# XuyangBai/D3Feat

Hardware: NVIDIA H100
Metric: points/sec through KPFCNN encoder (higher is better)
Workload: dtype f32

## Files before the change

d3feat_b200/csrc/kpconv.cu:

```cuda
#include <stdlib.h>

#include "ops.cuh"

namespace d3f {


constexpr int kS1Warps = 4;
constexpr int kWStride = 20;
constexpr int kKMax = 16;

struct Stage1Params {
  const float* q;
  const float4* s4;
  const int* idx;
  const float* feat;
  int count_nn;
  const float* Kp;
  const float* offsets;
  const float* modulations;
  int Nq, Ns, H, Cin;
  int n0, n1;
  const int* order;
  float extent;
  float inv_scale;
  float gauss_inv;
  int influence, closest;
  float shadow;
  float* wf;
  float* inv_nn;
  const int* nq_dev;
  const int* ns_dev;
};

__global__ void __launch_bounds__(256) prep_supports_kernel(const float* __restrict__ s, const float* __restrict__ feat,
                                                            int Ns_cap, const int* __restrict__ ns_dev, int Cin,
                                                            int mode, float shadow, float4* __restrict__ s4) {
  const int Ns = dyn_rows(Ns_cap, ns_dev);
  int warp = (blockIdx.x * blockDim.x + threadIdx.x) >> 5, lane = threadIdx.x & 31;
  if (warp > Ns) return;
  if (warp == Ns) {
    if (lane == 0) s4[Ns] = make_float4(shadow, shadow, shadow, 0.f);
    return;
  }
  float w = 0.f;
  if (mode == 1) {
    float sum = 0.f;
    for (int c = lane; c < Cin; c += 32) sum += feat[(size_t)warp * Cin + c];
#pragma unroll
    for (int o = 16; o > 0; o >>= 1) sum += __shfl_xor_sync(0xffffffffu, sum, o);
    w = sum > 0.f ? 1.f : 0.f;
  } else if (mode == 2) {
    w = feat[warp];
  }
  if (lane == 0) s4[warp] = make_float4(s[3 * (size_t)warp], s[3 * (size_t)warp + 1], s[3 * (size_t)warp + 2], w);
}

template <int G>
__global__ void __launch_bounds__(256) prep_supports_vec_kernel(const float* __restrict__ s,
                                                                const float* __restrict__ feat, int Ns_cap,
                                                                const int* __restrict__ ns_dev, int Cin,
                                                                float shadow, float4* __restrict__ s4) {
  const int Ns = dyn_rows(Ns_cap, ns_dev);
  const int t = blockIdx.x * blockDim.x + threadIdx.x;
  const int row = t / G, gl = t % G;
  float sum = 0.f;
  if (row < Ns) {
    const float4* fr = reinterpret_cast<const float4*>(feat + (size_t)row * Cin);
    for (int c4 = gl; c4 < Cin / 4; c4 += G) {
      float4 v = fr[c4];
      sum += (v.x + v.y) + (v.z + v.w);
    }
  }
#pragma unroll
  for (int o = G / 2; o > 0; o >>= 1) sum += __shfl_xor_sync(0xffffffffu, sum, o);
  if (gl == 0) {
    if (row < Ns)
      s4[row] = make_float4(s[3 * (size_t)row], s[3 * (size_t)row + 1], s[3 * (size_t)row + 2], sum > 0.f ? 1.f : 0.f);
    else if (row == Ns)
      s4[Ns] = make_float4(shadow, shadow, shadow, 0.f);
  }
}

template <int K, int VEC, bool DEFORM>
__global__ void __launch_bounds__(kS1Warps * 32) kpconv_stage1_kernel(Stage1Params p) {
  const int Ns_ = dyn_rows(p.Ns, p.ns_dev), n1_ = min(p.n1, dyn_rows(p.Nq, p.nq_dev));
  static_assert(K <= kKMax, "K too large");
  __shared__ __align__(16) float wts[kS1Warps][32 * kWStride];
  __shared__ float kp_s[kS1Warps][kKMax * 3];
  const int lane = threadIdx.x & 31, warp = threadIdx.x >> 5;
  const int n = p.n0 + blockIdx.x * kS1Warps + warp;
  if (n >= n1_) return;
  const int qid = p.order ? p.order[n] : n;

  for (int t = lane; t < K * 3; t += 32) {
    float v = p.Kp[t];
    if (DEFORM) v += p.offsets[(size_t)qid * K * 3 + t];
    kp_s[warp][t] = v;
  }
  for (int t = K * 3 + lane; t < kKMax * 3; t += 32) kp_s[warp][t] = 0.f;
  const float qx = p.q[3 * (size_t)qid], qy = p.q[3 * (size_t)qid + 1], qz = p.q[3 * (size_t)qid + 2];
  const int* row = p.idx + (size_t)qid * p.H;
  const float ext2 = p.extent * p.extent;
  __syncwarp();

  int nn_count = 0;
  const int c_step = 32 * VEC;
  for (int c0 = 0; c0 < p.Cin; c0 += c_step) {
    float acc[K][VEC];
#pragma unroll
    for (int k = 0; k < K; ++k)
#pragma unroll
      for (int v = 0; v < VEC; ++v) acc[k][v] = 0.f;
    const int c = c0 + lane * VEC;
    const bool c_ok = c < p.Cin;

    for (int h0 = 0; h0 < p.H; h0 += 32) {
      const int h = h0 + lane;
      int id = (h < p.H) ? row[h] : Ns_;
      if (id < 0 || id > Ns_) id = Ns_;
      const bool real = id < Ns_;
      const float4 sp = __ldg(&p.s4[id]);
      const float rx = sp.x - qx, ry = sp.y - qy, rz = sp.z - qz;
      float w[kKMax];
      float dmin = 3.0e38f;
      int kmin = 0;
      bool in_range = false;
#pragma unroll
      for (int k = 0; k < K; ++k) {
        float dx = rx - kp_s[warp][3 * k], dy = ry - kp_s[warp][3 * k + 1], dz = rz - kp_s[warp][3 * k + 2];
        float d2 = dx * dx + dy * dy + dz * dz;
        if (d2 < dmin) { dmin = d2; kmin = k; }
        in_range = in_range || (d2 < ext2);
        float wk;
        if (p.influence == D3F_INFLUENCE_LINEAR) wk = fmaxf(1.f - sqrtf(d2 + 1e-10f) * p.inv_scale, 0.f);
        else if (p.influence == D3F_INFLUENCE_GAUSSIAN) wk = expf(-d2 * p.gauss_inv);
        else wk = DEFORM ? (d2 < ext2 ? 1.f : 0.f) : 1.f;
        w[k] = wk;
      }
      if (p.closest) {
#pragma unroll
        for (int k = 0; k < K; ++k) w[k] = (k == kmin) ? w[k] : 0.f;
      }
      const bool keep = real && (!DEFORM || in_range);
#pragma unroll
      for (int k = 0; k < kKMax; ++k) wts[warp][lane * kWStride + k] = (keep && k < K) ? w[k] : 0.f;
      if (c0 == 0 && p.count_nn) nn_count += __popc(__ballot_sync(0xffffffffu, sp.w > 0.f));
      const unsigned keep_mask = __ballot_sync(0xffffffffu, keep);
      __syncwarp();

      unsigned m = keep_mask;
      while (m) {
        int hh[4];
        float f[4][VEC];
        int cnt = 0;
#pragma unroll
        for (int u = 0; u < 4; ++u) {
          if (m) {
            hh[u] = __ffs(m) - 1;
            m &= m - 1;
            ++cnt;
          } else {
            hh[u] = -1;
          }
        }
#pragma unroll
        for (int u = 0; u < 4; ++u) {
          if (hh[u] >= 0) {
            int idh = __shfl_sync(0xffffffffu, id, hh[u]);
            const float* fp = p.feat + (size_t)idh * p.Cin + c;
            if (VEC == 4) {
              float4 t = c_ok ? *reinterpret_cast<const float4*>(fp) : make_float4(0.f, 0.f, 0.f, 0.f);
              f[u][0] = t.x; f[u][1 % VEC] = t.y; f[u][2 % VEC] = t.z; f[u][3 % VEC] = t.w;
            } else if (VEC == 2) {
              float2 t = c_ok ? *reinterpret_cast<const float2*>(fp) : make_float2(0.f, 0.f);
              f[u][0] = t.x; f[u][1 % VEC] = t.y;
            } else {
              f[u][0] = c_ok ? *fp : 0.f;
            }
          }
        }
#pragma unroll
        for (int u = 0; u < 4; ++u) {
          if (hh[u] >= 0) {
            const float4* wp = reinterpret_cast<const float4*>(&wts[warp][hh[u] * kWStride]);
            float wv[kKMax];
#pragma unroll
            for (int kq = 0; kq < (K + 3) / 4; ++kq) {
              float4 t = wp[kq];
              wv[4 * kq] = t.x; wv[4 * kq + 1] = t.y; wv[4 * kq + 2] = t.z; wv[4 * kq + 3] = t.w;
            }
#pragma unroll
            for (int k = 0; k < K; ++k)
#pragma unroll
              for (int v = 0; v < VEC; ++v) acc[k][v] = fmaf(wv[k], f[u][v], acc[k][v]);
          }
        }
        (void)cnt;
      }
      __syncwarp();
    }

    if (c_ok) {
      float* dst = p.wf + (size_t)(n - p.n0) * K * p.Cin + c;
#pragma unroll
      for (int k = 0; k < K; ++k) {
        float mod = (DEFORM && p.modulations) ? p.modulations[(size_t)qid * K + k] : 1.f;
        if (VEC == 4) {
// ... 508 lines not shown
        mma_tf32(acc[i], ah, bl0, bl1);
      }
    }

    float* dst = p.wf + (size_t)(n - p.n0) * K * p.Cin + c0 + 2 * NT * t;
    const float modA = (DEFORM && p.modulations) ? p.modulations[(size_t)qid * K + kA] : 1.f;
    const float modB = (DEFORM && p.modulations && validB) ? p.modulations[(size_t)qid * K + kB] : 1.f;
#pragma unroll
    for (int v = 0; v < NT; v += 4) {
      *reinterpret_cast<float4*>(dst + (size_t)kA * p.Cin + v) =
          make_float4(acc[v][0] * modA, acc[v + 1][0] * modA, acc[v + 2][0] * modA, acc[v + 3][0] * modA);
      *reinterpret_cast<float4*>(dst + (size_t)kA * p.Cin + NT + v) =
          make_float4(acc[v][1] * modA, acc[v + 1][1] * modA, acc[v + 2][1] * modA, acc[v + 3][1] * modA);
      if (validB) {
        *reinterpret_cast<float4*>(dst + (size_t)kB * p.Cin + v) =
            make_float4(acc[v][2] * modB, acc[v + 1][2] * modB, acc[v + 2][2] * modB, acc[v + 3][2] * modB);
        *reinterpret_cast<float4*>(dst + (size_t)kB * p.Cin + NT + v) =
            make_float4(acc[v][3] * modB, acc[v + 1][3] * modB, acc[v + 2][3] * modB, acc[v + 3][3] * modB);
      }
    }
  }
  if (p.inv_nn != nullptr && lane == 0) p.inv_nn[n - p.n0] = 1.f / (float)max(nn_count, 1);
}

constexpr int kAnyKMax = 64;

template <bool DEFORM>
__global__ void __launch_bounds__(kS1Warps * 32) kpconv_stage1_anyk_kernel(Stage1Params p, int K) {
  const int Ns_ = dyn_rows(p.Ns, p.ns_dev), n1_ = min(p.n1, dyn_rows(p.Nq, p.nq_dev));
  extern __shared__ float anyk_smem[];
  const int lane = threadIdx.x & 31, warp = threadIdx.x >> 5;
  float* wts = anyk_smem + (size_t)warp * (K * 32 + K * 3);
  float* kp_s = wts + K * 32;
  const int n = p.n0 + blockIdx.x * kS1Warps + warp;
  if (n >= n1_) return;
  const int qid = p.order ? p.order[n] : n;
  for (int t = lane; t < K * 3; t += 32) {
    float v = p.Kp[t];
    if (DEFORM) v += p.offsets[(size_t)qid * K * 3 + t];
    kp_s[t] = v;
  }
  const float qx = p.q[3 * (size_t)qid], qy = p.q[3 * (size_t)qid + 1], qz = p.q[3 * (size_t)qid + 2];
  const int* row = p.idx + (size_t)qid * p.H;
  const float ext2 = p.extent * p.extent;
  float* dst = p.wf + (size_t)(n - p.n0) * K * p.Cin;
  __syncwarp();
  int nn_count = 0;
  for (int h0 = 0; h0 < p.H || h0 == 0; h0 += 32) {
    const int h = h0 + lane;
    int id = (h < p.H) ? row[h] : Ns_;
    if (id < 0 || id > Ns_) id = Ns_;
    const bool real = id < Ns_;
    const float4 sp = __ldg(&p.s4[id]);
    const float rx = sp.x - qx, ry = sp.y - qy, rz = sp.z - qz;
    float dmin = 3.0e38f;
    int kmin = 0;
    bool in_range = false;
    for (int k = 0; k < K; ++k) {
      float dx = rx - kp_s[3 * k], dy = ry - kp_s[3 * k + 1], dz = rz - kp_s[3 * k + 2];
      float d2 = dx * dx + dy * dy + dz * dz;
      if (d2 < dmin) { dmin = d2; kmin = k; }
      in_range = in_range || (d2 < ext2);
      float wk;
      if (p.influence == D3F_INFLUENCE_LINEAR) wk = fmaxf(1.f - sqrtf(d2 + 1e-10f) * p.inv_scale, 0.f);
      else if (p.influence == D3F_INFLUENCE_GAUSSIAN) wk = expf(-d2 * p.gauss_inv);
      else wk = DEFORM ? (d2 < ext2 ? 1.f : 0.f) : 1.f;
      wts[k * 32 + lane] = wk;
    }
    const bool keep = real && (!DEFORM || in_range);
    for (int k = 0; k < K; ++k) {
      float wk = wts[k * 32 + lane];
      if (p.closest && k != kmin) wk = 0.f;
      if (!keep) wk = 0.f;
      if (DEFORM && p.modulations) wk *= p.modulations[(size_t)qid * K + k];
      wts[k * 32 + lane] = wk;
    }
    if (p.count_nn) nn_count += __popc(__ballot_sync(0xffffffffu, sp.w > 0.f));
    const unsigned keep_mask = __ballot_sync(0xffffffffu, keep);
    __syncwarp();
    for (int c0 = 0; c0 < p.Cin; c0 += 32) {
      const int c = c0 + lane;
      const bool c_ok = c < p.Cin;
      for (int k = 0; k < K; ++k) {
        float acc = (h0 == 0 || !c_ok) ? 0.f : dst[(size_t)k * p.Cin + c];
        unsigned m = keep_mask;
        while (m) {
          const int j = __ffs(m) - 1;
          m &= m - 1;
          const int idj = __shfl_sync(0xffffffffu, id, j);
          if (c_ok) acc = fmaf(wts[k * 32 + j], p.feat[(size_t)idj * p.Cin + c], acc);
        }
        if (c_ok) dst[(size_t)k * p.Cin + c] = acc;
      }
    }
    __syncwarp();
  }
  if (p.inv_nn != nullptr && lane == 0) p.inv_nn[n - p.n0] = 1.f / (float)max(nn_count, 1);
}

template <bool DEFORM>
static int launch_stage1(int K, const Stage1Params& p, cudaStream_t stream) {
  int nq = p.n1 - p.n0;
  bool al16 = (reinterpret_cast<uintptr_t>(p.feat) & 15) == 0 && (reinterpret_cast<uintptr_t>(p.wf) & 15) == 0;
  if (K == 15 && al16 && (p.Cin == 32 || p.Cin == 64 || p.Cin % 128 == 0)) {
    const int blocks = ceil_div(nq, kS1Warps);
    const bool fast = p.influence == D3F_INFLUENCE_LINEAR && !p.closest;
    static const bool no_pared = [] { const char* v = getenv("D3F_S1_PARED"); return v != nullptr && v[0] == '0'; }();
    if (fast && !DEFORM && !no_pared && (long long)(p.Ns + 1) * p.Cin < (1ll << 31)) {
      const char* sv = getenv("D3F_S1_STAGED");
      const int staged = sv ? atoi(sv) : 0;
      const dim3 grid_wide(blocks, p.Cin >= 128 ? p.Cin / 64 : 1);
      if (staged) {
        if (p.Cin == 32) kpconv_stage1_staged_kernel<4><<<blocks, kS1Warps * 32, 0, stream>>>(p);
        else kpconv_stage1_staged_kernel<8><<<grid_wide, kS1Warps * 32, 0, stream>>>(p);
        D3F_LAUNCH_CHECK("kpconv_stage1_staged_kernel");
        return D3F_OK;
      }
      if (p.Cin == 32) kpconv_stage1_fast_kernel<4><<<blocks, kS1Warps * 32, 0, stream>>>(p);
      else kpconv_stage1_fast_kernel<8><<<grid_wide, kS1Warps * 32, 0, stream>>>(p);
      D3F_LAUNCH_CHECK("kpconv_stage1_fast_kernel");
      return D3F_OK;
    }
    if (fast) {
      if (p.Cin == 32) kpconv_stage1_mma_kernel<4, DEFORM, true><<<blocks, kS1Warps * 32, 0, stream>>>(p);
      else if (p.Cin == 64) kpconv_stage1_mma_kernel<8, DEFORM, true><<<blocks, kS1Warps * 32, 0, stream>>>(p);
      else kpconv_stage1_mma_kernel<16, DEFORM, true><<<blocks, kS1Warps * 32, 0, stream>>>(p);
    } else {
      if (p.Cin == 32) kpconv_stage1_mma_kernel<4, DEFORM, false><<<blocks, kS1Warps * 32, 0, stream>>>(p);
      else if (p.Cin == 64) kpconv_stage1_mma_kernel<8, DEFORM, false><<<blocks, kS1Warps * 32, 0, stream>>>(p);
      else kpconv_stage1_mma_kernel<16, DEFORM, false><<<blocks, kS1Warps * 32, 0, stream>>>(p);
    }
    D3F_LAUNCH_CHECK("kpconv_stage1_mma_kernel");
    return D3F_OK;
  }
  if (K == 15 && al16 && p.Cin % 64 == 0) {
    kpconv_stage1_v2_kernel<2, 1, DEFORM><<<ceil_div(nq, kS1Warps), kS1Warps * 32, 0, stream>>>(p);
  } else if (K == 15 && al16 && p.Cin % 32 == 0) {
    kpconv_stage1_v2_kernel<2, 2, DEFORM><<<ceil_div(nq, kS1Warps * 2), kS1Warps * 32, 0, stream>>>(p);
  } else if (K == 15) {
    kpconv_stage1_kernel<15, 1, DEFORM><<<ceil_div(nq, kS1Warps), kS1Warps * 32, 0, stream>>>(p);
  } else {
    const size_t smem = (size_t)kS1Warps * (K * 32 + K * 3) * sizeof(float);
    kpconv_stage1_anyk_kernel<DEFORM><<<ceil_div(nq, kS1Warps), kS1Warps * 32, smem, stream>>>(p, K);
  }
  D3F_LAUNCH_CHECK("kpconv_stage1_kernel");
  return D3F_OK;
}

struct Cin1Params {
  const float* q; const float4* s4; const int* idx; const float* Kp; const float* W;
  int Nq, Ns, H, Cout;
  float inv_scale, gauss_inv;
  int influence, closest, normalize;
  float shadow;
  const float* bn_scale; const float* bn_shift; const float* bias;
  float leaky_alpha;
  const int* order;
  float* out;
  const int* nq_dev; const int* ns_dev;
};

template <bool FAST>
__global__ void __launch_bounds__(256, 3) kpconv_cin1_kernel(Cin1Params p) {
  const int Ns_ = dyn_rows(p.Ns, p.ns_dev), Nq_ = dyn_rows(p.Nq, p.nq_dev);
  constexpr int K = 15;
  extern __shared__ float c1_smem[];
  float* Ws = c1_smem;
  float* kp_s = c1_smem + K * p.Cout;
  for (int t = threadIdx.x; t < K * p.Cout; t += blockDim.x) Ws[t] = p.W[t];
  for (int t = threadIdx.x; t < K * 3; t += blockDim.x) kp_s[t] = p.Kp[t];
  __syncthreads();
  const int lane = threadIdx.x & 31;
  const int sub = lane >> 3, sl = lane & 7;
  const int slot0 = ((blockIdx.x * blockDim.x + threadIdx.x) >> 5) * 4;
  if (slot0 >= Nq_) return;
  const int slot = slot0 + sub;
  const bool qvalid = slot < Nq_;
  const int n = p.order ? p.order[qvalid ? slot : slot0] : (qvalid ? slot : slot0);
  const float qx = p.q[3 * (size_t)n], qy = p.q[3 * (size_t)n + 1], qz = p.q[3 * (size_t)n + 2];
  const int* row = p.idx + (size_t)n * p.H;
  float wf[K];
#pragma unroll
  for (int k = 0; k < K; ++k) wf[k] = 0.f;
  int nn = 0;
  if (FAST) {
    float kp[K * 3];
#pragma unroll
    for (int i = 0; i < K * 3; ++i) kp[i] = kp_s[i];
    const float inv_scale = p.inv_scale;
    const unsigned Nsu = (unsigned)Ns_;
    unsigned id1 = Nsu, id2 = Nsu;
    if (sl < p.H) id1 = min((unsigned)__ldg(row + sl), Nsu);
    if (sl + 8 < p.H) id2 = min((unsigned)__ldg(row + sl + 8), Nsu);
    float4 sp_n = __ldg(&p.s4[id1]);
    for (int h = sl; h < p.H; h += 8) {
      const float4 sp = sp_n;
      sp_n = __ldg(&p.s4[id2]);
      id2 = Nsu;
      if (h + 16 < p.H) id2 = min((unsigned)__ldg(row + h + 16), Nsu);
      const float f = sp.w, rx = sp.x - qx, ry = sp.y - qy, rz = sp.z - qz;
      nn += f > 0.f ? 1 : 0;
#pragma unroll
      for (int k = 0; k < K; ++k) {
        const float dx = rx - kp[3 * k], dy = ry - kp[3 * k + 1], dz = rz - kp[3 * k + 2];
        const float d2 = fmaf(dz, dz, fmaf(dy, dy, fmaf(dx, dx, 1e-10f)));
        const float wk = fmaxf(fmaf(-sqrt_approx(d2), inv_scale, 1.f), 0.f);
        wf[k] = fmaf(wk, f, wf[k]);
      }
    }
  } else
  for (int h = sl; h < p.H; h += 8) {
    int id = row[h];
    if (id < 0 || id > Ns_) id = Ns_;
    const float4 sp = __ldg(&p.s4[id]);
    const float f = sp.w, rx = sp.x - qx, ry = sp.y - qy, rz = sp.z - qz;
    nn += f > 0.f ? 1 : 0;
    float w[K];
    float dmin = 3.0e38f;
    int kmin = 0;
#pragma unroll
    for (int k = 0; k < K; ++k) {
      float dx = rx - kp_s[3 * k], dy = ry - kp_s[3 * k + 1], dz = rz - kp_s[3 * k + 2];
      float d2 = dx * dx + dy * dy + dz * dz;
      if (d2 < dmin) { dmin = d2; kmin = k; }
      float wk;
      if (p.influence == D3F_INFLUENCE_LINEAR) wk = fmaxf(1.f - sqrt_approx(d2 + 1e-10f) * p.inv_scale, 0.f);
      else if (p.influence == D3F_INFLUENCE_GAUSSIAN) wk = __expf(-d2 * p.gauss_inv);
      else wk = 1.f;
      w[k] = wk;
    }
#pragma unroll
    for (int k = 0; k < K; ++k) wf[k] += (p.closest && k != kmin) ? 0.f : w[k] * f;
  }
#pragma unroll
  for (int o = 1; o < 8; o <<= 1) {
#pragma unroll
    for (int k = 0; k < K; ++k) wf[k] += __shfl_xor_sync(0xffffffffu, wf[k], o);
    nn += __shfl_xor_sync(0xffffffffu, nn, o);
  }
  if (!qvalid) return;
  const float inv_nn = p.normalize ? 1.f / (float)max(nn, 1) : 1.f;
  for (int c = sl; c < p.Cout; c += 8) {
    float y = 0.f;
#pragma unroll
    for (int k = 0; k < K; ++k) y = fmaf(wf[k], Ws[k * p.Cout + c], y);
    y *= inv_nn;
    if (p.bn_scale) y = fmaf(y, p.bn_scale[c], p.bn_shift[c]);
    if (p.bias) y += p.bias[c];
    if (p.leaky_alpha >= 0.f) y = y > 0.f ? y : y * p.leaky_alpha;
    p.out[(size_t)n * p.Cout + c] = y;
  }
}

struct AuxStream {
  cudaStream_t stream = nullptr;
  cudaEvent_t s1_done[2] = {nullptr, nullptr};
  cudaEvent_t gemm_done[2] = {nullptr, nullptr};
};
constexpr int kMaxDevices = 32;
struct AuxStreams {
  AuxStream dev[kMaxDevices];
  ~AuxStreams() {
    for (int d = 0; d < kMaxDevices; ++d) {
      if (dev[d].stream == nullptr) continue;
      int cur = 0;
      if (cudaGetDevice(&cur) != cudaSuccess || cudaSetDevice(d) != cudaSuccess) continue;
      for (int i = 0; i < 2; ++i) {
        cudaEventDestroy(dev[d].s1_done[i]);
        cudaEventDestroy(dev[d].gemm_done[i]);
      }
      cudaStreamDestroy(dev[d].stream);
      cudaSetDevice(cur);
    }
  }
};
static AuxStream* aux_stream() {
  static thread_local AuxStreams all;
  int dev = 0;
  if (cudaGetDevice(&dev) != cudaSuccess || dev < 0 || dev >= kMaxDevices) return nullptr;
  AuxStream& a = all.dev[dev];
  if (a.stream != nullptr) return &a;
  cudaStreamCaptureMode mode = cudaStreamCaptureModeRelaxed;
  cudaThreadExchangeStreamCaptureMode(&mode);
  AuxStream n;
  bool ok = cudaStreamCreateWithFlags(&n.stream, cudaStreamNonBlocking) == cudaSuccess;
  for (int i = 0; ok && i < 2; ++i)
    ok = cudaEventCreateWithFlags(&n.s1_done[i], cudaEventDisableTiming) == cudaSuccess &&
         cudaEventCreateWithFlags(&n.gemm_done[i], cudaEventDisableTiming) == cudaSuccess;
  cudaThreadExchangeStreamCaptureMode(&mode);
  if (!ok) return nullptr;
  a = n;
  return &a;
}

static int chunk_queries(int K, int Cin) {
  static const int forced = [] { const char* v = getenv("D3F_KPCONV_CHUNK"); return v ? atoi(v) : 0; }();
  if (forced >= 128) return forced / 128 * 128;
  const long long per = (long long)K * Cin * 4;
  long long n = (512ll << 20) / per;
  if (n < 1024) n = 1024;
  return (int)(n / 128 * 128);
}

int kpconv_chunk_queries(int K, int Cin) { return chunk_queries(K, Cin); }

int kpconv_prep_supports(bool deform, const float* s, const float* feat, int Ns, const int* ns_dev, int K, int Cin,
                         int normalize, float4* s4, cudaStream_t stream) {
  const bool norm = normalize != 0 && !deform;
  const bool first_layer = Cin == 1 && !deform && K == 15;
  int pmode = first_layer ? 2 : (norm ? 1 : 0);
  const float shadow = deform ? 1000.f : 1e6f;
  const bool vec = pmode == 1 && Cin % 4 == 0 && Cin >= 32 && (reinterpret_cast<uintptr_t>(feat) & 15) == 0;
  if (vec && Cin < 64)
    prep_supports_vec_kernel<8><<<ceil_div((Ns + 1) * 8, 256), 256, 0, stream>>>(s, feat, Ns, ns_dev, Cin, shadow, s4);
  else if (vec && Cin < 128)
    prep_supports_vec_kernel<16><<<ceil_div((Ns + 1) * 16, 256), 256, 0, stream>>>(s, feat, Ns, ns_dev, Cin, shadow, s4);
  else if (vec)
    prep_supports_vec_kernel<32><<<ceil_div((Ns + 1) * 32, 256), 256, 0, stream>>>(s, feat, Ns, ns_dev, Cin, shadow, s4);
  else
    prep_supports_kernel<<<ceil_div((Ns + 1) * 32, 256), 256, 0, stream>>>(s, feat, Ns, ns_dev, Cin, pmode, shadow, s4);
  D3F_LAUNCH_CHECK("prep_supports_kernel");
  return D3F_OK;
}

int kpconv_stage1_wf(const float* q, const float4* s4, const int* idx, const float* feat, const float* Kp, int Nq, int Ns,
                     int H, int K, int Cin, float extent, int influence, int mode, int n0, int n1, float* wf,
                     cudaStream_t stream, const int* nq_dev, const int* ns_dev) {
  Stage1Params p;
  p.q = q; p.s4 = s4; p.idx = idx; p.feat = feat; p.count_nn = 0;
  p.Kp = Kp; p.offsets = nullptr; p.modulations = nullptr;
  p.Nq = Nq; p.Ns = Ns; p.H = H; p.Cin = Cin;
  p.n0 = n0; p.n1 = n1;
  p.order = nullptr;
  p.extent = extent;
  p.inv_scale = 1.f / (2.f * extent);
  float sigma = extent * 0.3f;
  p.gauss_inv = 1.f / (2.f * sigma * sigma + 1e-9f);
  p.influence = influence;
  p.closest = mode == D3F_MODE_CLOSEST;
  p.shadow = 1e6f;
  p.wf = wf;
  p.inv_nn = nullptr;
  p.nq_dev = nq_dev; p.ns_dev = ns_dev;
  return launch_stage1<false>(K, p, stream);
}

struct KpconvWs {
  float* wf[2];
  float* nn[2];
  float4* s4;
  float* split;
  float* w_img;
};

static size_t kpconv_layout(int Nq, int Ns, int K, int Cin, int Cout, void* base, KpconvWs* w_out) {
  int chunk = chunk_queries(K, Cin);
  if (chunk > Nq) chunk = Nq > 0 ? Nq : 1;
  Carver cv(base);
  KpconvWs w;
  for (int b = 0; b < 2; ++b) w.wf[b] = cv.take<float>((size_t)chunk * K * Cin);
  for (int b = 0; b < 2; ++b) w.nn[b] = cv.take<float>(chunk);
  w.s4 = cv.take<float4>((size_t)Ns + 1);
  const size_t split_floats = tc_gemm_split_ws_floats(chunk, Cout, K * Cin);
  w.split = split_floats ? cv.take<float>(split_floats) : nullptr;
  w.w_img = cv.take<float>(kpconv_fused_image_floats());
  if (w_out != nullptr) *w_out = w;
  return cv.off;
}

int kpconv_forward_impl(bool deform, const float* q, const float* s, const int* idx, const float* feat,
                        const float* Kp, const float* offsets, const float* modulations, const float* W,
                        const float* W_packed, const int* query_order, int Nq, int Ns, int H, int K, int Cin, int Cout,
                        float extent,
                        int influence, int mode, int normalize,
                        const float* bn_scale, const float* bn_shift, const float* bias, float leaky_alpha,
                        float* out, void* workspace, size_t workspace_bytes, cudaStream_t stream,
                        const int* nq_dev, const int* ns_dev) {
  D3F_REQUIRE(Nq >= 0 && Ns >= 0 && H >= 0 && Cin >= 1 && Cout >= 1, D3F_ERR_INVALID,
              "kpconv: bad shape Nq=%d Ns=%d H=%d Cin=%d Cout=%d", Nq, Ns, H, Cin, Cout);
  D3F_REQUIRE(K >= 1 && K <= kAnyKMax, D3F_ERR_INVALID, "kpconv: num_kernel_points=%d outside [1, %d]", K, kAnyKMax);
  D3F_REQUIRE(influence >= 0 && influence <= 2, D3F_ERR_INVALID,
              "Unknown influence function type (config.KP_influence)");
  D3F_REQUIRE(mode == D3F_MODE_SUM || mode == D3F_MODE_CLOSEST, D3F_ERR_INVALID,
              "Unknown convolution mode. Should be 'closest' or 'sum'");
  D3F_REQUIRE(extent > 0.f, D3F_ERR_INVALID, "kpconv: KP_extent=%g", (double)extent);
  D3F_REQUIRE((bn_scale == nullptr) == (bn_shift == nullptr), D3F_ERR_INVALID, "kpconv: bn_scale/bn_shift mismatch");
  D3F_REQUIRE(!deform || offsets != nullptr || Nq == 0, D3F_ERR_INVALID, "kpconv_deform: offsets missing");
  KpconvWs w;
  const size_t need = kpconv_layout(Nq, Ns, K, Cin, Cout, workspace, &w);
  D3F_REQUIRE(need > 0 && workspace_bytes >= need, D3F_ERR_WORKSPACE, "kpconv: workspace too small");
  if (Nq == 0) return D3F_OK;
  int chunk = chunk_queries(K, Cin);
  if (chunk > Nq) chunk = Nq;
  float4* s4 = w.s4;
  const bool norm = normalize != 0 && !deform;
  {
    const int rc = kpconv_prep_supports(deform, s, feat, Ns, ns_dev, K, Cin, normalize, s4, stream);
    if (rc) return rc;
  }
  const size_t c1_smem = (size_t)(K * Cout + K * 3) * sizeof(float);
  if (Cin == 1 && !deform && K == 15 && c1_smem <= 48 * 1024) {
    Cin1Params c1;
    c1.q = q; c1.s4 = s4; c1.idx = idx; c1.Kp = Kp; c1.W = W;
    c1.Nq = Nq; c1.Ns = Ns; c1.H = H; c1.Cout = Cout;
    c1.inv_scale = 1.f / (2.f * extent);
    float sg = extent * 0.3f;
    c1.gauss_inv = 1.f / (2.f * sg * sg + 1e-9f);
    c1.influence = influence; c1.closest = mode == D3F_MODE_CLOSEST; c1.normalize = normalize != 0;
    c1.shadow = 1e6f;
    c1.bn_scale = bn_scale; c1.bn_shift = bn_shift; c1.bias = bias; c1.leaky_alpha = leaky_alpha;
    c1.order = query_order;
    c1.out = out;
    c1.nq_dev = nq_dev; c1.ns_dev = ns_dev;
    if (influence == D3F_INFLUENCE_LINEAR && mode == D3F_MODE_SUM)
      kpconv_cin1_kernel<true><<<ceil_div(ceil_div(Nq, 4) * 32, 256), 256, c1_smem, stream>>>(c1);
    else
      kpconv_cin1_kernel<false><<<ceil_div(ceil_div(Nq, 4) * 32, 256), 256, c1_smem, stream>>>(c1);
    D3F_LAUNCH_CHECK("kpconv_cin1_kernel");
    return D3F_OK;
  }
  if (!deform && W_packed != nullptr &&
      kpconv_fused_supported(Nq, H, K, Cin, Cout, influence, mode, feat, W, out, query_order)) {
    return kpconv_fused_forward(q, s4, idx, feat, Kp, W, w.w_img, Nq, Ns, H, Cout, extent, norm ? 1 : 0, bn_scale, bn_shift,
                                bias, leaky_alpha, out, stream, nq_dev, ns_dev);
  }
  Stage1Params p;
  p.q = q; p.s4 = s4; p.idx = idx; p.feat = feat; p.count_nn = norm ? 1 : 0;
  p.Kp = Kp; p.offsets = offsets; p.modulations = modulations;
  p.Nq = Nq; p.Ns = Ns; p.H = H; p.Cin = Cin;
  p.extent = extent;
  p.inv_scale = deform ? 1.f / extent : 1.f / (2.f * extent);
  float sigma = extent * 0.3f;
  p.gauss_inv = 1.f / (2.f * sigma * sigma + 1e-9f);
  p.influence = influence;
  p.closest = mode == D3F_MODE_CLOSEST;
  p.shadow = deform ? 1000.f : 1e6f;
  p.order = query_order;
  p.nq_dev = nq_dev; p.ns_dev = ns_dev;
  const int n_chunks = ceil_div(Nq, chunk);
  AuxStream* aux = n_chunks > 1 ? aux_stream() : nullptr;
  for (int ci = 0, n0 = 0; n0 < Nq; n0 += chunk, ++ci) {
    const int b = ci & 1;
    float* wf = w.wf[b];
    float* inv_nn = w.nn[b];
    p.wf = wf;
    p.inv_nn = norm ? inv_nn : nullptr;
    p.n0 = n0;
    p.n1 = min(Nq, n0 + chunk);
    if (aux && ci >= 2) D3F_CUDA(cudaStreamWaitEvent(stream, aux->gemm_done[b], 0));
    int rc = deform ? launch_stage1<true>(K, p, stream) : launch_stage1<false>(K, p, stream);
    if (rc) return rc;
    cudaStream_t gs = stream;
    if (aux) {
      D3F_CUDA(cudaEventRecord(aux->s1_done[b], stream));
      D3F_CUDA(cudaStreamWaitEvent(aux->stream, aux->s1_done[b], 0));
      gs = aux->stream;
    }
    Epilogue ep;
    ep.rowscale = norm ? inv_nn : nullptr;
    ep.bn_scale = bn_scale; ep.bn_shift = bn_shift; ep.bias = bias; ep.residual = nullptr;
    ep.leaky_alpha = leaky_alpha;
    ep.row_map = query_order ? query_order + n0 : nullptr;
    ep.m_dev = nq_dev; ep.m_off = n0;
    float* cbase = query_order ? out : out + (size_t)n0 * Cout;
    if (W_packed != nullptr && tc_gemm_supported(wf, K * Cin))
      rc = tc_gemm(wf, W_packed, cbase, p.n1 - n0, Cout, K * Cin, ep, gs, w.split);
    else
      rc = gemm_f32(wf, W, cbase, p.n1 - n0, Cout, K * Cin, ep, gs);
    if (rc) return rc;
    if (aux) D3F_CUDA(cudaEventRecord(aux->gemm_done[b], aux->stream));
  }
  if (aux) {
    D3F_CUDA(cudaStreamWaitEvent(stream, aux->gemm_done[0], 0));
    if (n_chunks > 1) D3F_CUDA(cudaStreamWaitEvent(stream, aux->gemm_done[1], 0));
  }
  return D3F_OK;
}

}

using namespace d3f;

extern "C" size_t d3f_kpconv_workspace_bytes(int Nq, int Ns, int H, int K, int Cin, int Cout) {
  (void)H;
  return kpconv_layout(Nq, Ns, K, Cin, Cout, nullptr, nullptr);
}

extern "C" int d3f_kpconv_forward(const float* q, const float* s, const int* idx, const float* feat, const float* Kp,
                                  const float* W, const float* W_packed, const int* query_order, int Nq, int Ns, int H,
                                  int K, int Cin, int Cout, float extent, int influence, int mode, int normalize,
                                  const float* bn_scale, const float* bn_shift, const float* bias, float leaky_alpha,
                                  float* out, void* workspace, size_t workspace_bytes, d3f_stream_t stream,
                                  const int* nq_dev, const int* ns_dev) {
  D3F_REQUIRE(Nq == 0 || (q && idx && Kp && W && out && workspace && (Ns == 0 || (s && feat))), D3F_ERR_INVALID,
              "d3f_kpconv_forward: null pointer");
  return kpconv_forward_impl(false, q, s, idx, feat, Kp, nullptr, nullptr, W, W_packed, query_order, Nq, Ns, H, K, Cin,
                             Cout, extent, influence, mode, normalize, bn_scale, bn_shift, bias, leaky_alpha, out,
                             workspace, workspace_bytes, (cudaStream_t)stream, nq_dev, ns_dev);
}

extern "C" int d3f_kpconv_deform_forward(const float* q, const float* s, const int* idx, const float* feat,
                                         const float* Kp, const float* offsets, const float* modulations,
                                         const float* W, const float* W_packed, const int* query_order, int Nq, int Ns,
                                         int H, int K, int Cin, int Cout, float extent, int influence, int mode,
                                         const float* bn_scale, const float* bn_shift, const float* bias,
                                         float leaky_alpha, float* out, void* workspace, size_t workspace_bytes,
                                         d3f_stream_t stream, const int* nq_dev, const int* ns_dev) {
  D3F_REQUIRE(Nq == 0 || (q && idx && Kp && W && out && workspace && offsets && (Ns == 0 || (s && feat))),
              D3F_ERR_INVALID, "d3f_kpconv_deform_forward: null pointer");
  return kpconv_forward_impl(true, q, s, idx, feat, Kp, offsets, modulations, W, W_packed, query_order, Nq, Ns, H, K,
                             Cin, Cout, extent, influence, mode, 0, bn_scale, bn_shift, bias, leaky_alpha, out,
                             workspace, workspace_bytes, (cudaStream_t)stream, nq_dev, ns_dev);
}
```

Before: 64.83 million.

## Restructure Cin=1 KPConv kernel as persistent grid with pipelined neighbor loads

The single-input-channel KPConv kernel becomes a persistent, grid-strided kernel sized to SM count. It prefetches the next query's neighbor indices and support points while the current query computes, and handles two neighbors per iteration. The warp reduction is replaced by a transpose-style shuffle reduce, followed by a shared-memory exchange. Weights are re-laid out in shared memory for float4 output computation and vectorized stores, larger Cout is allowed through opt-in shared memory, and a lightweight per-row prep kernel is added for the non-summing modes. The change adds register pressure and code complexity, and cudaGetDevice and cudaDeviceGetAttribute are now called on every launch.

```diff
diff --git a/d3feat_b200/csrc/kpconv.cu b/d3feat_b200/csrc/kpconv.cu
--- a/d3feat_b200/csrc/kpconv.cu
+++ b/d3feat_b200/csrc/kpconv.cu
@@ -32,9 +32,21 @@
   const int* ns_dev;
 };
 
+__global__ void __launch_bounds__(256) prep_supports_rows_kernel(const float* __restrict__ s,
+                                                                 const float* __restrict__ feat, int Ns_cap,
+                                                                 const int* __restrict__ ns_dev, int with_feat,
+                                                                 float shadow, float4* __restrict__ s4) {
+  const int Ns = dyn_rows(Ns_cap, ns_dev);
+  const int i = blockIdx.x * blockDim.x + threadIdx.x;
+  if (i < Ns)
+    s4[i] = make_float4(s[3 * (size_t)i], s[3 * (size_t)i + 1], s[3 * (size_t)i + 2], with_feat ? feat[i] : 0.f);
+  else if (i == Ns)
+    s4[Ns] = make_float4(shadow, shadow, shadow, 0.f);
+}
+
 __global__ void __launch_bounds__(256) prep_supports_kernel(const float* __restrict__ s, const float* __restrict__ feat,
                                                             int Ns_cap, const int* __restrict__ ns_dev, int Cin,
-                                                            int mode, float shadow, float4* __restrict__ s4) {
+                                                            float shadow, float4* __restrict__ s4) {
   const int Ns = dyn_rows(Ns_cap, ns_dev);
   int warp = (blockIdx.x * blockDim.x + threadIdx.x) >> 5, lane = threadIdx.x & 31;
   if (warp > Ns) return;
@@ -42,17 +54,13 @@
     if (lane == 0) s4[Ns] = make_float4(shadow, shadow, shadow, 0.f);
     return;
   }
-  float w = 0.f;
-  if (mode == 1) {
-    float sum = 0.f;
-    for (int c = lane; c < Cin; c += 32) sum += feat[(size_t)warp * Cin + c];
-#pragma unroll
-    for (int o = 16; o > 0; o >>= 1) sum += __shfl_xor_sync(0xffffffffu, sum, o);
-    w = sum > 0.f ? 1.f : 0.f;
-  } else if (mode == 2) {
-    w = feat[warp];
-  }
-  if (lane == 0) s4[warp] = make_float4(s[3 * (size_t)warp], s[3 * (size_t)warp + 1], s[3 * (size_t)warp + 2], w);
+  float sum = 0.f;
+  for (int c = lane; c < Cin; c += 32) sum += feat[(size_t)warp * Cin + c];
+#pragma unroll
+  for (int o = 16; o > 0; o >>= 1) sum += __shfl_xor_sync(0xffffffffu, sum, o);
+  if (lane == 0)
+    s4[warp] = make_float4(s[3 * (size_t)warp], s[3 * (size_t)warp + 1], s[3 * (size_t)warp + 2],
+                           sum > 0.f ? 1.f : 0.f);
 }
 
 template <int G>
@@ -867,7 +875,7 @@
   int Nq, Ns, H, Cout;
   float inv_scale, gauss_inv;
   int influence, closest, normalize;
-  float shadow;
+  int vec;
   const float* bn_scale; const float* bn_shift; const float* bias;
   float leaky_alpha;
   const int* order;
@@ -875,95 +883,212 @@
   const int* nq_dev; const int* ns_dev;
 };
 
+constexpr int kC1Warps = 8;
+constexpr int kC1Blocks = 4;
+constexpr int kC1MaxCout = 816;
+
+static inline size_t cin1_smem_floats(int K, int Cout) {
+  return (size_t)(Cout + 3) / 4 * 4 * K + 4 * K + kC1Warps * 64;
+}
+
+__device__ __forceinline__ float cin1_linear(float rx, float ry, float rz, const float4& kp, float inv_scale) {
+  const float dx = rx - kp.x, dy = ry - kp.y, dz = rz - kp.z;
+  const float d2 = fmaf(dz, dz, fmaf(dy, dy, fmaf(dx, dx, 1e-10f)));
+  return fmaxf(fmaf(-sqrt_approx(d2), inv_scale, 1.f), 0.f);
+}
+
 template <bool FAST>
-__global__ void __launch_bounds__(256, 3) kpconv_cin1_kernel(Cin1Params p) {
+__global__ void __launch_bounds__(kC1Warps * 32, kC1Blocks) kpconv_cin1_kernel(Cin1Params p) {
+  constexpr int K = 15;
   const int Ns_ = dyn_rows(p.Ns, p.ns_dev), Nq_ = dyn_rows(p.Nq, p.nq_dev);
-  constexpr int K = 15;
-  extern __shared__ float c1_smem[];
+  extern __shared__ __align__(16) float c1_smem[];
+  const int Cout = p.Cout, H = p.H;
   float* Ws = c1_smem;
-  float* kp_s = c1_smem + K * p.Cout;
-  for (int t = threadIdx.x; t < K * p.Cout; t += blockDim.x) Ws[t] = p.W[t];
-  for (int t = threadIdx.x; t < K * 3; t += blockDim.x) kp_s[t] = p.Kp[t];
+  float4* kp_s = reinterpret_cast<float4*>(c1_smem + (Cout + 3) / 4 * 4 * K);
+  for (int t = threadIdx.x; t < K * Cout; t += blockDim.x) {
+    const int k = t / Cout, c = t - k * Cout;
+    Ws[((c >> 2) * K + k) * 4 + (c & 3)] = p.W[t];
+  }
+  if (threadIdx.x < K)
+    kp_s[threadIdx.x] = make_float4(p.Kp[3 * threadIdx.x], p.Kp[3 * threadIdx.x + 1], p.Kp[3 * threadIdx.x + 2], 0.f);
   __syncthreads();
-  const int lane = threadIdx.x & 31;
+  const int lane = threadIdx.x & 31, warp = threadIdx.x >> 5;
   const int sub = lane >> 3, sl = lane & 7;
-  const int slot0 = ((blockIdx.x * blockDim.x + threadIdx.x) >> 5) * 4;
-  if (slot0 >= Nq_) return;
-  const int slot = slot0 + sub;
-  const bool qvalid = slot < Nq_;
-  const int n = p.order ? p.order[qvalid ? slot : slot0] : (qvalid ? slot : slot0);
-  const float qx = p.q[3 * (size_t)n], qy = p.q[3 * (size_t)n + 1], qz = p.q[3 * (size_t)n + 2];
-  const int* row = p.idx + (size_t)n * p.H;
-  float wf[K];
-#pragma unroll
-  for (int k = 0; k < K; ++k) wf[k] = 0.f;
-  int nn = 0;
-  if (FAST) {
-    float kp[K * 3];
-#pragma unroll
-    for (int i = 0; i < K * 3; ++i) kp[i] = kp_s[i];
-    const float inv_scale = p.inv_scale;
-    const unsigned Nsu = (unsigned)Ns_;
-    unsigned id1 = Nsu, id2 = Nsu;
-    if (sl < p.H) id1 = min((unsigned)__ldg(row + sl), Nsu);
-    if (sl + 8 < p.H) id2 = min((unsigned)__ldg(row + sl + 8), Nsu);
-    float4 sp_n = __ldg(&p.s4[id1]);
-    for (int h = sl; h < p.H; h += 8) {
-      const float4 sp = sp_n;
-      sp_n = __ldg(&p.s4[id2]);
-      id2 = Nsu;
-      if (h + 16 < p.H) id2 = min((unsigned)__ldg(row + h + 16), Nsu);
-      const float f = sp.w, rx = sp.x - qx, ry = sp.y - qy, rz = sp.z - qz;
-      nn += f > 0.f ? 1 : 0;
-#pragma unroll
-      for (int k = 0; k < K; ++k) {
-        const float dx = rx - kp[3 * k], dy = ry - kp[3 * k + 1], dz = rz - kp[3 * k + 2];
-        const float d2 = fmaf(dz, dz, fmaf(dy, dy, fmaf(dx, dx, 1e-10f)));
-        const float wk = fmaxf(fmaf(-sqrt_approx(d2), inv_scale, 1.f), 0.f);
-        wf[k] = fmaf(wk, f, wf[k]);
-      }
-    }
-  } else
-  for (int h = sl; h < p.H; h += 8) {
-    int id = row[h];
-    if (id < 0 || id > Ns_) id = Ns_;
-    const float4 sp = __ldg(&p.s4[id]);
-    const float f = sp.w, rx = sp.x - qx, ry = sp.y - qy, rz = sp.z - qz;
-    nn += f > 0.f ? 1 : 0;
-    float w[K];
-    float dmin = 3.0e38f;
-    int kmin = 0;
-#pragma unroll
-    for (int k = 0; k < K; ++k) {
-      float dx = rx - kp_s[3 * k], dy = ry - kp_s[3 * k + 1], dz = rz - kp_s[3 * k + 2];
-      float d2 = dx * dx + dy * dy + dz * dz;
-      if (d2 < dmin) { dmin = d2; kmin = k; }
-      float wk;
-      if (p.influence == D3F_INFLUENCE_LINEAR) wk = fmaxf(1.f - sqrt_approx(d2 + 1e-10f) * p.inv_scale, 0.f);
-      else if (p.influence == D3F_INFLUENCE_GAUSSIAN) wk = __expf(-d2 * p.gauss_inv);
-      else wk = 1.f;
-      w[k] = wk;
-    }
-#pragma unroll
-    for (int k = 0; k < K; ++k) wf[k] += (p.closest && k != kmin) ? 0.f : w[k] * f;
-  }
-#pragma unroll
-  for (int o = 1; o < 8; o <<= 1) {
-#pragma unroll
-    for (int k = 0; k < K; ++k) wf[k] += __shfl_xor_sync(0xffffffffu, wf[k], o);
-    nn += __shfl_xor_sync(0xffffffffu, nn, o);
-  }
-  if (!qvalid) return;
-  const float inv_nn = p.normalize ? 1.f / (float)max(nn, 1) : 1.f;
-  for (int c = sl; c < p.Cout; c += 8) {
-    float y = 0.f;
-#pragma unroll
-    for (int k = 0; k < K; ++k) y = fmaf(wf[k], Ws[k * p.Cout + c], y);
-    y *= inv_nn;
-    if (p.bn_scale) y = fmaf(y, p.bn_scale[c], p.bn_shift[c]);
-    if (p.bias) y += p.bias[c];
-    if (p.leaky_alpha >= 0.f) y = y > 0.f ? y : y * p.leaky_alpha;
-    p.out[(size_t)n * p.Cout + c] = y;
+  float* xs = reinterpret_cast<float*>(kp_s + K) + warp * 64 + sub * 16;
+  const int groups = (Nq_ + 3) >> 2;
+  const int stride = gridDim.x * kC1Warps;
+  int g = blockIdx.x * kC1Warps + warp;
+  if (g >= groups) return;
+
+  const unsigned Nsu = (unsigned)Ns_;
+  const int pairs = (H + 15) >> 4;
+  const bool odd = ((H + 7) >> 3) & 1;
+  auto query = [&](int grp) {
+    const int slot = grp * 4 + sub;
+    const int sv = slot < Nq_ ? slot : grp * 4;
+    return p.order ? __ldg(p.order + sv) : sv;
+  };
+  auto nb = [&](const int* row, int j) {
+    const int h = sl + 8 * j;
+    return h < H ? min((unsigned)__ldg(row + h), Nsu) : Nsu;
+  };
+  auto row_of = [&](int n) { return p.idx + (size_t)n * H; };
+  const float inv_scale = p.inv_scale;
+
+  int n = query(g);
+  float qx = __ldg(p.q + 3 * (size_t)n), qy = __ldg(p.q + 3 * (size_t)n + 1), qz = __ldg(p.q + 3 * (size_t)n + 2);
+  const int* row = row_of(n);
+  unsigned idA = nb(row, 0), idB = nb(row, 1);
+  float4 spA = __ldg(&p.s4[idA]), spB = __ldg(&p.s4[idB]);
+  idA = nb(row, 2); idB = nb(row, 3);
+  for (;;) {
+    const int gn = g + stride;
+    const bool next = gn < groups;
+    const int n_next = next ? query(gn) : 0;
+    float v[16];
+#pragma unroll
+    for (int k = 0; k < 16; ++k) v[k] = 0.f;
+    for (int t = 0; t < pairs; ++t) {
+      const float4 a = spA, b = spB;
+      if (t + 1 < pairs) {
+        spA = __ldg(&p.s4[idA]);
+        spB = __ldg(&p.s4[idB]);
+        idA = nb(row, 2 * t + 4);
+        idB = nb(row, 2 * t + 5);
+      } else if (next) {
+        row = row_of(n_next);
+        idA = nb(row, 0);
+        idB = nb(row, 1);
+      }
+      const bool two = t + 1 < pairs || !odd;
+      const float ax = a.x - qx, ay = a.y - qy, az = a.z - qz, fa = a.w;
+      const float bx = b.x - qx, by = b.y - qy, bz = b.z - qz, fb = b.w;
+      v[15] += fa > 0.f ? 1.f : 0.f;
+      if (two) v[15] += fb > 0.f ? 1.f : 0.f;
+      if (FAST) {
+        if (two) {
+#pragma unroll
+          for (int k = 0; k < K; ++k) {
+            const float4 kp = kp_s[k];
+            v[k] = fmaf(cin1_linear(ax, ay, az, kp, inv_scale), fa, v[k]);
+            v[k] = fmaf(cin1_linear(bx, by, bz, kp, inv_scale), fb, v[k]);
+          }
+        } else {
+#pragma unroll
+          for (int k = 0; k < K; ++k) v[k] = fmaf(cin1_linear(ax, ay, az, kp_s[k], inv_scale), fa, v[k]);
+        }
+      } else {
+#pragma unroll 1
+        for (int e = 0; e < (two ? 2 : 1); ++e) {
+          const float rx = e ? bx : ax, ry = e ? by : ay, rz = e ? bz : az, f = e ? fb : fa;
+          auto dist2 = [&](int k) {
+            const float4 kp = kp_s[k];
+            const float dx = rx - kp.x, dy = ry - kp.y, dz = rz - kp.z;
+            return dx * dx + dy * dy + dz * dz;
+          };
+          int kmin = 0;
+          if (p.closest) {
+            float dmin = 3.0e38f;
+            for (int k = 0; k < K; ++k) {
+              const float d2 = dist2(k);
+              if (d2 < dmin) { dmin = d2; kmin = k; }
+            }
+          }
+#pragma unroll
+          for (int k = 0; k < K; ++k) {
+            const float d2 = dist2(k);
+            float wk;
+            if (p.influence == D3F_INFLUENCE_LINEAR) wk = fmaxf(1.f - sqrt_approx(d2 + 1e-10f) * p.inv_scale, 0.f);
+            else if (p.influence == D3F_INFLUENCE_GAUSSIAN) wk = __expf(-d2 * p.gauss_inv);
+            else wk = 1.f;
+            v[k] += (p.closest && k != kmin) ? 0.f : wk * f;
+          }
+        }
+      }
+    }
+    const int n_cur = n;
+    if (next) {
+      spA = __ldg(&p.s4[idA]);
+      spB = __ldg(&p.s4[idB]);
+      if (pairs == 0) row = row_of(n_next);
+      idA = nb(row, 2);
+      idB = nb(row, 3);
+      qx = __ldg(p.q + 3 * (size_t)n_next);
+      qy = __ldg(p.q + 3 * (size_t)n_next + 1);
+      qz = __ldg(p.q + 3 * (size_t)n_next + 2);
+    }
+    {
+      const bool b0 = sl & 1, b1 = sl & 2, b2 = sl & 4;
+#pragma unroll
+      for (int j = 0; j < 8; ++j) {
+        const float send = b0 ? v[j] : v[j + 8], keep = b0 ? v[j + 8] : v[j];
+        v[j] = keep + __shfl_xor_sync(0xffffffffu, send, 1);
+      }
+#pragma unroll
+      for (int j = 0; j < 4; ++j) {
+        const float send = b1 ? v[j] : v[j + 4], keep = b1 ? v[j + 4] : v[j];
+        v[j] = keep + __shfl_xor_sync(0xffffffffu, send, 2);
+      }
+#pragma unroll
+      for (int j = 0; j < 2; ++j) {
+        const float send = b2 ? v[j] : v[j + 2], keep = b2 ? v[j + 2] : v[j];
+        v[j] = keep + __shfl_xor_sync(0xffffffffu, send, 4);
+      }
+      __syncwarp();
+      *reinterpret_cast<float2*>(xs + (b0 ? 8 : 0) + (b1 ? 4 : 0) + (b2 ? 2 : 0)) = make_float2(v[0], v[1]);
+      __syncwarp();
+#pragma unroll
+      for (int j = 0; j < 4; ++j) {
+        const float4 x = reinterpret_cast<const float4*>(xs)[j];
+        v[4 * j] = x.x; v[4 * j + 1] = x.y; v[4 * j + 2] = x.z; v[4 * j + 3] = x.w;
+      }
+    }
+    if (g * 4 + sub < Nq_) {
+      const float inv_nn = p.normalize ? 1.f / fmaxf(v[15], 1.f) : 1.f;
+      const float alpha = p.leaky_alpha;
+      float* orow = p.out + (size_t)n_cur * Cout;
+      if (p.vec) {
+        for (int c = 4 * sl; c < Cout; c += 32) {
+          float4 y = make_float4(0.f, 0.f, 0.f, 0.f);
+#pragma unroll
+          for (int k = 0; k < K; ++k) {
+            const float4 w = reinterpret_cast<const float4*>(Ws)[(c >> 2) * K + k];
+            y.x = fmaf(v[k], w.x, y.x); y.y = fmaf(v[k], w.y, y.y);
+            y.z = fmaf(v[k], w.z, y.z); y.w = fmaf(v[k], w.w, y.w);
+          }
+          y.x *= inv_nn; y.y *= inv_nn; y.z *= inv_nn; y.w *= inv_nn;
+          if (p.bn_scale) {
+            const float4 s = __ldg(reinterpret_cast<const float4*>(p.bn_scale + c));
+            const float4 b = __ldg(reinterpret_cast<const float4*>(p.bn_shift + c));
+            y.x = fmaf(y.x, s.x, b.x); y.y = fmaf(y.y, s.y, b.y); y.z = fmaf(y.z, s.z, b.z); y.w = fmaf(y.w, s.w, b.w);
+          }
+          if (p.bias) {
+            const float4 b = __ldg(reinterpret_cast<const float4*>(p.bias + c));
+            y.x += b.x; y.y += b.y; y.z += b.z; y.w += b.w;
+          }
+          if (alpha >= 0.f) {
+            y.x = y.x > 0.f ? y.x : y.x * alpha; y.y = y.y > 0.f ? y.y : y.y * alpha;
+            y.z = y.z > 0.f ? y.z : y.z * alpha; y.w = y.w > 0.f ? y.w : y.w * alpha;
+          }
+          *reinterpret_cast<float4*>(orow + c) = y;
+        }
+      } else {
+        for (int c = sl; c < Cout; c += 8) {
+          float y = 0.f;
+          const float* wq = Ws + (c >> 2) * K * 4 + (c & 3);
+#pragma unroll
+          for (int k = 0; k < K; ++k) y = fmaf(v[k], wq[4 * k], y);
+          y *= inv_nn;
+          if (p.bn_scale) y = fmaf(y, __ldg(p.bn_scale + c), __ldg(p.bn_shift + c));
+          if (p.bias) y += __ldg(p.bias + c);
+          if (alpha >= 0.f) y = y > 0.f ? y : y * alpha;
+          orow[c] = y;
+        }
+      }
+    }
+    if (!next) break;
+    g = gn;
+    n = n_next;
   }
 }
 
@@ -1032,8 +1157,10 @@
     prep_supports_vec_kernel<16><<<ceil_div((Ns + 1) * 16, 256), 256, 0, stream>>>(s, feat, Ns, ns_dev, Cin, shadow, s4);
   else if (vec)
     prep_supports_vec_kernel<32><<<ceil_div((Ns + 1) * 32, 256), 256, 0, stream>>>(s, feat, Ns, ns_dev, Cin, shadow, s4);
+  else if (pmode == 1)
+    prep_supports_kernel<<<ceil_div((Ns + 1) * 32, 256), 256, 0, stream>>>(s, feat, Ns, ns_dev, Cin, shadow, s4);
   else
-    prep_supports_kernel<<<ceil_div((Ns + 1) * 32, 256), 256, 0, stream>>>(s, feat, Ns, ns_dev, Cin, pmode, shadow, s4);
+    prep_supports_rows_kernel<<<ceil_div(Ns + 1, 256), 256, 0, stream>>>(s, feat, Ns, ns_dev, pmode == 2, shadow, s4);
   D3F_LAUNCH_CHECK("prep_supports_kernel");
   return D3F_OK;
 }
@@ -1113,8 +1240,7 @@
     const int rc = kpconv_prep_supports(deform, s, feat, Ns, ns_dev, K, Cin, normalize, s4, stream);
     if (rc) return rc;
   }
-  const size_t c1_smem = (size_t)(K * Cout + K * 3) * sizeof(float);
-  if (Cin == 1 && !deform && K == 15 && c1_smem <= 48 * 1024) {
+  if (Cin == 1 && !deform && K == 15 && Cout <= kC1MaxCout) {
     Cin1Params c1;
     c1.q = q; c1.s4 = s4; c1.idx = idx; c1.Kp = Kp; c1.W = W;
     c1.Nq = Nq; c1.Ns = Ns; c1.H = H; c1.Cout = Cout;
@@ -1122,15 +1248,28 @@
     float sg = extent * 0.3f;
     c1.gauss_inv = 1.f / (2.f * sg * sg + 1e-9f);
     c1.influence = influence; c1.closest = mode == D3F_MODE_CLOSEST; c1.normalize = normalize != 0;
-    c1.shadow = 1e6f;
+    auto al16 = [](const float* ptr) { return (reinterpret_cast<uintptr_t>(ptr) & 15) == 0; };
+    c1.vec = Cout % 4 == 0 && al16(out) && al16(bn_scale) && al16(bn_shift) && al16(bias);
     c1.bn_scale = bn_scale; c1.bn_shift = bn_shift; c1.bias = bias; c1.leaky_alpha = leaky_alpha;
     c1.order = query_order;
     c1.out = out;
     c1.nq_dev = nq_dev; c1.ns_dev = ns_dev;
-    if (influence == D3F_INFLUENCE_LINEAR && mode == D3F_MODE_SUM)
-      kpconv_cin1_kernel<true><<<ceil_div(ceil_div(Nq, 4) * 32, 256), 256, c1_smem, stream>>>(c1);
+    const size_t smem = cin1_smem_floats(K, Cout) * sizeof(float);
+    int dev = 0, sms = 0;
+    D3F_CUDA(cudaGetDevice(&dev));
+    D3F_CUDA(cudaDeviceGetAttribute(&sms, cudaDevAttrMultiProcessorCount, dev));
+    int blocks = ceil_div(ceil_div(Nq, 4), kC1Warps);
+    if (blocks > sms * kC1Blocks) blocks = sms * kC1Blocks;
+    const bool fast = influence == D3F_INFLUENCE_LINEAR && mode == D3F_MODE_SUM;
+    if (smem > 48 * 1024) {
+      const int most = (int)(cin1_smem_floats(K, kC1MaxCout) * sizeof(float));
+      if (fast) D3F_CUDA(cudaFuncSetAttribute(kpconv_cin1_kernel<true>, cudaFuncAttributeMaxDynamicSharedMemorySize, most));
+      else D3F_CUDA(cudaFuncSetAttribute(kpconv_cin1_kernel<false>, cudaFuncAttributeMaxDynamicSharedMemorySize, most));
+    }
+    if (fast)
+      kpconv_cin1_kernel<true><<<blocks, kC1Warps * 32, smem, stream>>>(c1);
     else
-      kpconv_cin1_kernel<false><<<ceil_div(ceil_div(Nq, 4) * 32, 256), 256, c1_smem, stream>>>(c1);
+      kpconv_cin1_kernel<false><<<blocks, kC1Warps * 32, smem, stream>>>(c1);
     D3F_LAUNCH_CHECK("kpconv_cin1_kernel");
     return D3F_OK;
   }
```

After: 66.02 million (median of 6 runs). 1.02x the previous value.
